# Jordy-VL/multi-modal-early-exit

Hardware: NVIDIA B200
Metric: docs/sec @ calibrated exit threshold (higher is better)
Workload: dtype bf16

## Files before the change

multi-modal-early-exit_b200/csrc/attention.cuh:

```cuda
#pragma once
#include <cuda.h>

#include <type_traits>

#include "ptx.cuh"

namespace mmee {

constexpr int ATT_SM_WARPS = 4;
constexpr int ATT_THREADS = 64 + ATT_SM_WARPS * 32;
constexpr int ATT_CTAS_PER_SM = 2;
constexpr int ATT_BQ = 128;
constexpr int ATT_BKV = 64;
constexpr int ATT_D = 64;
constexpr int ATT_DV = 80;
constexpr int ATT_KB_STAGES = 2;
constexpr int ATT_V_STAGES = 2;
constexpr int ATT_MAX_KV_TILES = 16;
constexpr float ATT_LAZY = 8.0f;
constexpr float ATT_JUMP = 40.0f;

template <bool kSplit>
struct AttSmemT {
  static constexpr int NP = kSplit ? 2 : 1;
  static constexpr int Q_BYTES = ATT_BQ * ATT_D * 2;
  static constexpr int K_BYTES = ATT_BKV * ATT_D * 2;
  static constexpr int V_BYTES = ATT_DV * ATT_BKV * 2;
  static constexpr int VLO_BYTES = kSplit ? ATT_D * ATT_BKV * 2 : 0;
  static constexpr int B_BYTES = ATT_BQ * ATT_BKV * 2;
  static constexpr int Q_STAGE = NP * Q_BYTES;
  static constexpr int KB_STAGE = NP * (K_BYTES + B_BYTES);
  static constexpr int V_STAGE = V_BYTES + VLO_BYTES;
  static constexpr int I_BYTES = ATT_BKV * ATT_BKV * 2;
  static constexpr int Q_OFF = 0;
  static constexpr int KB_OFF = Q_OFF + 2 * Q_STAGE;
  static constexpr int V_OFF = KB_OFF + ATT_KB_STAGES * KB_STAGE;
  static constexpr int I_OFF = V_OFF + ATT_V_STAGES * V_STAGE;
  static constexpr int BAR_OFF = I_OFF + I_BYTES;
  static constexpr int N_BARS = 2 + 2 + 2 * ATT_KB_STAGES + 2 * ATT_V_STAGES + 2 + 2 + 1 + 1;
  static constexpr int TOTAL = BAR_OFF + N_BARS * 8 + 16;
  static constexpr int DYN_BYTES = TOTAL;
  static constexpr uint32_t TMEM_COLS = kSplit ? 512 : 256;
};
using AttSmem = AttSmemT<false>;
static_assert(AttSmem::DYN_BYTES <= 115712, "two attention CTAs must fit one SM");
static_assert(AttSmemT<true>::DYN_BYTES <= 232448, "split attention CTA must fit one SM");
static_assert(AttSmem::KB_STAGE % 1024 == 0 && AttSmem::K_BYTES % 1024 == 0 && AttSmem::V_BYTES % 1024 == 0 &&
                  AttSmem::V_OFF % 1024 == 0 && AttSmem::I_OFF % 1024 == 0 && AttSmemT<true>::V_STAGE % 1024 == 0 &&
                  AttSmemT<true>::V_OFF % 1024 == 0 && AttSmemT<true>::I_OFF % 1024 == 0,
              "swizzled tiles need 1024 B alignment");

struct AttArgs {
  const int4* slot_meta;
  const int* qt_slot;
  const int* n_qt_dev;
  int* err_flag;
  long long* trace;
  __nv_bfloat16* ctx;
  __nv_bfloat16* ctx_lo;
  int H, heads, seq;
  int tail16;
  int experiment;
};

__device__ __forceinline__ float fast_exp2(float x) {
  float y;
  asm("ex2.approx.ftz.f32 %0, %1;" : "=f"(y) : "f"(x));
  return y;
}

__device__ __forceinline__ void sub_ref_x2(uint32_t a, uint32_t b, uint64_t nref2, float& ya, float& yb) {
  uint64_t x, y;
  asm("mov.b64 %0, {%1, %2};" : "=l"(x) : "r"(a), "r"(b));
  asm("add.rn.f32x2 %0, %1, %2;" : "=l"(y) : "l"(x), "l"(nref2));
  asm("mov.b64 {%0, %1}, %2;" : "=f"(ya), "=f"(yb) : "l"(y));
}

// ... 16 lines not shown
  c.nitem = total_items;
  if (!c.valid) return c;
  c.row0 = meta.x; c.rows = meta.y; c.doc = meta.z;
  const int n_qt = (c.rows + ATT_BQ - 1) / ATT_BQ;
  const int local = item - args.heads * meta.w;
  c.head = local / n_qt;
  c.q0 = (local - c.head * n_qt) * ATT_BQ;
  c.slot = __ldg(args.qt_slot + item / args.heads);
  c.last_j = (c.rows + ATT_BKV - 1) / ATT_BKV - 1;
  const int rem = c.rows - c.last_j * ATT_BKV;
  c.tail_j = (args.tail16 && c.last_j > 0 && rem <= 16) ? c.last_j : -1;
  c.nitem = item + stride;
  c.nmeta = att_item_meta(c.nitem, total_items, args);
  return c;
}
__device__ __forceinline__ AttCursor att_first(int total_items, int stride, const AttArgs& args) {
  const int item = blockIdx.x;
  return att_enter(item, 0, att_item_meta(item, total_items, args), total_items, stride, args);
}
__device__ __forceinline__ AttCursor att_next(AttCursor c, int total_items, int stride, const AttArgs& args) {
  if (c.j < c.last_j) { ++c.j; return c; }
  return att_enter(c.nitem, c.ii + 1, c.nmeta, total_items, stride, args);
}

struct AttMaps {
  CUtensorMap q, k, vt, bias, q_lo, k_lo, vt_lo, bias_lo;
};

template <bool kTrace, bool kSplit = false>
__global__ void __launch_bounds__(ATT_THREADS, kSplit ? 1 : ATT_CTAS_PER_SM)
attention_kernel(const __grid_constant__ AttMaps maps, const AttArgs args) {
  using SMEM = AttSmemT<kSplit>;
  const CUtensorMap& tmap_q = maps.q;
  const CUtensorMap& tmap_k = maps.k;
  const CUtensorMap& tmap_vt = maps.vt;
  const CUtensorMap& tmap_bias = maps.bias;
  const int S = args.seq;
  const int total_items = *args.n_qt_dev * args.heads;
  const int stride = gridDim.x;
  if (total_items == 0) return;

  extern __shared__ __align__(1024) uint8_t smem_raw[];
  const uint32_t sb = smem_u32(smem_raw);
  uint8_t* smem = smem_raw;
  if (sb & 1023u) __trap();
  const uint32_t bar0 = sb + SMEM::BAR_OFF;
  const uint32_t q_full = bar0;
  const uint32_t q_empty = q_full + 2 * 8;
  const uint32_t kb_full = q_empty + 2 * 8;
  const uint32_t kb_empty = kb_full + ATT_KB_STAGES * 8;
  const uint32_t v_full = kb_empty + ATT_KB_STAGES * 8;
  const uint32_t v_empty = v_full + ATT_V_STAGES * 8;
  const uint32_t s_full = v_empty + ATT_V_STAGES * 8;
  const uint32_t p_full = s_full + 2 * 8;
  const uint32_t o_full = p_full + 2 * 8;
  const uint32_t qt_full = o_full + 8;
  uint64_t* bars = reinterpret_cast<uint64_t*>(smem + SMEM::BAR_OFF);
  uint32_t* tmem_slot = reinterpret_cast<uint32_t*>(bars + SMEM::N_BARS);

  const int warp = threadIdx.x >> 5;
  const int lane = threadIdx.x & 31;
#define ATT_TRACE(R, T, K)                                                                             \
  if constexpr (kTrace) {                                                                              \
    if (blockIdx.x == 0 && (T) < 96) args.trace[(R) * 1024 + (T) * 8 + (K)] = clock64();              \
  }

  if (warp == 0 && lane == 0) {
    tma_prefetch_desc(&tmap_q);
    tma_prefetch_desc(&tmap_k);
    tma_prefetch_desc(&tmap_vt);
    tma_prefetch_desc(&tmap_bias);
    if constexpr (kSplit) {
      tma_prefetch_desc(&maps.q_lo); tma_prefetch_desc(&maps.k_lo); tma_prefetch_desc(&maps.vt_lo); tma_prefetch_desc(&maps.bias_lo);
    }
    uint64_t* b = bars;
    for (int i = 0; i < 2; ++i) mbar_init(b++, 1);
    for (int i = 0; i < 2; ++i) mbar_init(b++, ATT_SM_WARPS);
    for (int i = 0; i < 2 * ATT_KB_STAGES; ++i) mbar_init(b++, 1);
    for (int i = 0; i < 2 * ATT_V_STAGES; ++i) mbar_init(b++, 1);
    for (int i = 0; i < 2; ++i) mbar_init(b++, 1);
    for (int i = 0; i < 2; ++i) mbar_init(b++, ATT_SM_WARPS);
    mbar_init(b++, 1);
    mbar_init(b++, ATT_SM_WARPS);
    fence_mbar_init();
  }
  for (int i = threadIdx.x; i < ATT_V_STAGES * 128; i += blockDim.x) {
    const int stg = i >> 7, chunk = i & 127;
    uint8_t* base = smem + SMEM::V_OFF + stg * SMEM::V_STAGE + ATT_D * 128;
    const uint32_t val = (chunk < 8) ? 0x3F803F80u : 0u;
    *reinterpret_cast<uint4*>(base + chunk * 16) = make_uint4(val, val, val, val);
  }
  for (int i = threadIdx.x; i < ATT_BKV * 8; i += blockDim.x) {
    const int n = i >> 3, cchunk = i & 7;
    uint32_t w[4] = {0u, 0u, 0u, 0u};
    if ((n >> 3) == cchunk) w[(n & 7) >> 1] = (n & 1) ? 0x3C000000u : 0x00003C00u;
    *reinterpret_cast<uint4*>(smem + SMEM::I_OFF + n * 128 + ((cchunk ^ (n & 7)) << 4)) = make_uint4(w[0], w[1], w[2], w[3]);
  }
  fence_proxy_async_smem();
  if (warp == 1) tmem_alloc<SMEM::TMEM_COLS>(tmem_slot);
  tc_fence_before();
  __syncthreads();
  tc_fence_after();
  const uint32_t tmem_base = *tmem_slot;
  const uint32_t tmem_S = tmem_base;
  const uint32_t tmem_O = tmem_base + 128;
  const uint32_t tmem_Q = tmem_base + 208;
  const uint32_t tmem_Qlo = tmem_base + 240;

  if (warp == 0) {
    if (elect_one()) {
      AttCursor c = att_first(total_items, stride, args);
      uint32_t t = 0;
      int loaded_ii = -1;
      int pv_row = 0, pv_kv0 = 0;
      constexpr int PF_DIST = 4;
      while (c.valid) {
        const int row0 = c.row0;
        if (c.ii != loaded_ii) {
          loaded_ii = c.ii;
          auto load_q = [&](int k, int qrow, int qhead) {
            const int qb = k & 1;
            mbar_wait(q_empty + qb * 8, ((k >> 1) & 1) ^ 1);
            mbar_expect_tx(q_full + qb * 8, SMEM::Q_STAGE);
            tma_load_2d(sb + SMEM::Q_OFF + qb * SMEM::Q_STAGE, &tmap_q, q_full + qb * 8, qhead * ATT_D, qrow);
            if constexpr (kSplit)
              tma_load_2d(sb + SMEM::Q_OFF + qb * SMEM::Q_STAGE + SMEM::Q_BYTES, &maps.q_lo, q_full + qb * 8, qhead * ATT_D, qrow);
          };
          ATT_TRACE(2, t, 2)
          if (c.ii == 0) load_q(0, row0 + c.q0, c.head);
          if (c.nitem < total_items) {
            const int nn_qt = (c.nmeta.y + ATT_BQ - 1) / ATT_BQ;
            const int nlocal = c.nitem - args.heads * c.nmeta.w;
            const int nhead = nlocal / nn_qt;
            load_q(c.ii + 1, c.nmeta.x + (nlocal - nhead * nn_qt) * ATT_BQ, nhead);
          }
        }
        const int kv0 = c.j * ATT_BKV;
        const int brow = (c.doc * args.heads + c.head) * S + c.q0;
        const int vrow = (c.slot * args.heads + c.head) * ATT_D;
        const int st = t % ATT_KB_STAGES;
        ATT_TRACE(2, t, 0)
        mbar_wait(kb_empty + st * 8, ((t / ATT_KB_STAGES) & 1) ^ 1);
        ATT_TRACE(2, t, 1)
        const uint32_t sk = sb + SMEM::KB_OFF + st * SMEM::KB_STAGE;
        if (!kSplit && args.experiment && t >= 4) {
          const uint32_t bytes = ((args.experiment & 1) ? 0 : SMEM::K_BYTES) + ((args.experiment & 2) ? 0 : SMEM::B_BYTES);
          if (bytes) mbar_expect_tx(kb_full + st * 8, bytes); else mbar_arrive(kb_full + st * 8);
          if (!(args.experiment & 1)) tma_load_2d(sk, &tmap_k, kb_full + st * 8, args.H + c.head * ATT_D, row0 + kv0);
          if (!(args.experiment & 2)) tma_load_2d(sk + SMEM::NP * SMEM::K_BYTES, &tmap_bias, kb_full + st * 8, kv0, brow);
        } else {
        mbar_expect_tx(kb_full + st * 8, SMEM::KB_STAGE);
        tma_load_2d(sk, &tmap_k, kb_full + st * 8, args.H + c.head * ATT_D, row0 + kv0);
        tma_load_2d(sk + SMEM::NP * SMEM::K_BYTES, &tmap_bias, kb_full + st * 8, kv0, brow);
        }
        if constexpr (kSplit) {
          tma_load_2d(sk + SMEM::K_BYTES, &maps.k_lo, kb_full + st * 8, args.H + c.head * ATT_D, row0 + kv0);
          tma_load_2d(sk + 2 * SMEM::K_BYTES + SMEM::B_BYTES, &maps.bias_lo, kb_full + st * 8, kv0, brow);
        }
        {
// ... 16 lines not shown
            }
          }
          if (pj <= plast) {
            tma_prefetch_2d(&tmap_bias, pj * ATT_BKV, pbrow);
            tma_prefetch_2d(&tmap_k, args.H + phead * ATT_D, prow0 + pj * ATT_BKV);
            tma_prefetch_2d(&tmap_vt, pj * ATT_BKV, pvrow);
          }
        }
        if (t > 0) {
          const int sv = (t - 1) % ATT_V_STAGES;
          mbar_wait(v_empty + sv * 8, (((t - 1) / ATT_V_STAGES) & 1) ^ 1);
          if (!kSplit && (args.experiment & 1) && t >= 4) {
            mbar_arrive(v_full + sv * 8);
          } else {
          mbar_expect_tx(v_full + sv * 8, SMEM::NP * ATT_D * ATT_BKV * 2);
          tma_load_2d(sb + SMEM::V_OFF + sv * SMEM::V_STAGE, &tmap_vt, v_full + sv * 8, pv_kv0, pv_row);
          if constexpr (kSplit)
            tma_load_2d(sb + SMEM::V_OFF + sv * SMEM::V_STAGE + SMEM::V_BYTES, &maps.vt_lo, v_full + sv * 8, pv_kv0, pv_row);
          }
        }
        pv_row = vrow; pv_kv0 = kv0;
        ++t;
        c = att_next(c, total_items, stride, args);
      }
      if (t > 0) {
        const int sv = (t - 1) % ATT_V_STAGES;
        mbar_wait(v_empty + sv * 8, (((t - 1) / ATT_V_STAGES) & 1) ^ 1);
        mbar_expect_tx(v_full + sv * 8, SMEM::NP * ATT_D * ATT_BKV * 2);
        tma_load_2d(sb + SMEM::V_OFF + sv * SMEM::V_STAGE, &tmap_vt, v_full + sv * 8, pv_kv0, pv_row);
        if constexpr (kSplit)
          tma_load_2d(sb + SMEM::V_OFF + sv * SMEM::V_STAGE + SMEM::V_BYTES, &maps.vt_lo, v_full + sv * 8, pv_kv0, pv_row);
      }
    }
  } else if (warp == 1) {
    if (elect_one()) {
      constexpr uint32_t idesc_s = umma_idesc_bf16(ATT_BQ, ATT_BKV);
      constexpr uint32_t idesc_o = umma_idesc_bf16(ATT_BQ, ATT_DV);
      constexpr uint32_t idesc_s16 = umma_idesc_bf16(ATT_BQ, 16);
      constexpr uint32_t idesc_b16 = umma_idesc_f16(ATT_BQ, 16);
      const uint64_t di = umma_desc_sw128_kmajor(sb + SMEM::I_OFF);
      AttCursor cs = att_first(total_items, stride, args);
      AttCursor cp = cs;
      uint32_t ts = 0;
      auto issue_s = [&]() {
        const int st = ts % ATT_KB_STAGES;
        ATT_TRACE(1, ts, 0)
        if (cs.j == 0) mbar_wait(qt_full, cs.ii & 1);
        mbar_wait(kb_full + st * 8, (ts / ATT_KB_STAGES) & 1);
        ATT_TRACE(1, ts, 1)
        tc_fence_after();
        const uint32_t stage = sb + SMEM::KB_OFF + st * SMEM::KB_STAGE;
        const uint64_t dk = umma_desc_sw128_kmajor(stage);
        const uint64_t db = umma_desc_sw128_kmajor(stage + SMEM::NP * SMEM::K_BYTES);
        const uint32_t d_s = tmem_S + (ts & 1) * ATT_BKV;
        if constexpr (kSplit) {
          const uint64_t dkl = umma_desc_sw128_kmajor(stage + SMEM::K_BYTES);
          const uint64_t dbl = umma_desc_sw128_kmajor(stage + 2 * SMEM::K_BYTES + SMEM::B_BYTES);
#pragma unroll
          for (int k = 0; k < ATT_D / 16; ++k) umma_bf16_ts(d_s, tmem_Q + k * 8, dk + 2 * k, idesc_s, k ? 1u : 0u);
#pragma unroll
          for (int k = 0; k < ATT_D / 16; ++k) umma_bf16_ts(d_s, tmem_Qlo + k * 8, dk + 2 * k, idesc_s, 1u);
#pragma unroll
          for (int k = 0; k < ATT_D / 16; ++k) umma_bf16_ts(d_s, tmem_Q + k * 8, dkl + 2 * k, idesc_s, 1u);
#pragma unroll
          for (int k = 0; k < ATT_BKV / 16; ++k) umma_bf16_ss(d_s + 16 * k, db + 2 * k, di + 130 * k, idesc_b16, 1u);
#pragma unroll
// ... 12 lines not shown
        umma_commit(kb_empty + st * 8);
        ++ts;
        cs = att_next(cs, total_items, stride, args);
      };
      if (cs.valid) issue_s();
      for (uint32_t t = 0; t < ts; ++t) {
        if (cs.valid) issue_s();
        const int sv = t % ATT_V_STAGES;
        const int b = t & 1;
        const bool first = (cp.j == 0);
        ATT_TRACE(1, t, 2)
        mbar_wait(p_full + b * 8, (t >> 1) & 1);
        ATT_TRACE(1, t, 3)
        mbar_wait(v_full + sv * 8, (t / ATT_V_STAGES) & 1);
        tc_fence_after();
        const uint64_t dv = umma_desc_sw128_kmajor(sb + SMEM::V_OFF + sv * SMEM::V_STAGE);
        const int pv_steps = (kSplit || cp.j != cp.tail_j) ? ATT_BKV / 16 : 1;
#pragma unroll
        for (int k = 0; k < ATT_BKV / 16; ++k)
          if (k < pv_steps)
            umma_bf16_ts(tmem_O, tmem_S + b * ATT_BKV + k * 8, dv + 2 * k, idesc_o, (k || !first) ? 1u : 0u);
        if constexpr (kSplit) {
          constexpr uint32_t idesc_o64 = umma_idesc_bf16(ATT_BQ, ATT_D);
          const uint64_t dvl = umma_desc_sw128_kmajor(sb + SMEM::V_OFF + sv * SMEM::V_STAGE + SMEM::V_BYTES);
#pragma unroll
          for (int k = 0; k < ATT_BKV / 16; ++k) umma_bf16_ts(tmem_O, tmem_S + b * ATT_BKV + 32 + k * 8, dv + 2 * k, idesc_o, 1u);
#pragma unroll
          for (int k = 0; k < ATT_BKV / 16; ++k) umma_bf16_ts(tmem_O, tmem_S + b * ATT_BKV + k * 8, dvl + 2 * k, idesc_o64, 1u);
        }
        umma_commit(o_full);
        umma_commit(v_empty + sv * 8);
        cp = att_next(cp, total_items, stride, args);
      }
    }
  } else {
    const int quarter = warp & 3;
    const int r = quarter * 32 + lane;
    const uint32_t lane_addr = static_cast<uint32_t>(quarter * 32) << 16;
    uint32_t t = 0;
    AttCursor c = att_first(total_items, stride, args);

    float ref = 0.f, alpha_pend = 1.f;
    __nv_bfloat16* out_ptr = nullptr;
    bool have_item = false;

    auto store_item = [&](__nv_bfloat16* dst_row) {
      uint32_t v[32];
      const uint32_t lsum = tmem_ld1(tmem_O + lane_addr + ATT_D);
      tmem_ld32(tmem_O + lane_addr, v);
      tmem_ld_wait();
      const float inv = 1.0f / __uint_as_float(lsum);
      if constexpr (kSplit) {
        __nv_bfloat16* lo_row = dst_row ? args.ctx_lo + (dst_row - args.ctx) : nullptr;
#pragma unroll
        for (int hh = 0; hh < 2; ++hh) {
// ... 28 lines not shown
      tmem_ld32(tmem_O + lane_addr + 32, v);
      tmem_ld_wait();
      if (dst_row) {
#pragma unroll
        for (int i = 0; i < 4; ++i)
          dst[4 + i] = make_uint4(pack_bf16x2(__uint_as_float(v[i * 8 + 0]) * inv, __uint_as_float(v[i * 8 + 1]) * inv),
                                  pack_bf16x2(__uint_as_float(v[i * 8 + 2]) * inv, __uint_as_float(v[i * 8 + 3]) * inv),
                                  pack_bf16x2(__uint_as_float(v[i * 8 + 4]) * inv, __uint_as_float(v[i * 8 + 5]) * inv),
                                  pack_bf16x2(__uint_as_float(v[i * 8 + 6]) * inv, __uint_as_float(v[i * 8 + 7]) * inv));
      }
    };

    auto q_to_tmem = [&](int ii) {
      const int qb = ii & 1;
      mbar_wait(q_full + qb * 8, (ii >> 1) & 1);
      const uint32_t qrow = sb + SMEM::Q_OFF + qb * SMEM::Q_STAGE + r * 128;
      uint32_t q[32];
#pragma unroll
      for (int cch = 0; cch < 8; ++cch) {
        const uint4 x = lds128(qrow + ((cch ^ (r & 7)) << 4));
        q[4 * cch] = x.x; q[4 * cch + 1] = x.y; q[4 * cch + 2] = x.z; q[4 * cch + 3] = x.w;
      }
      tmem_st32(tmem_Q + lane_addr, q);
      if constexpr (kSplit) {
#pragma unroll
        for (int cch = 0; cch < 8; ++cch) {
          const uint4 x = lds128(qrow + SMEM::Q_BYTES + ((cch ^ (r & 7)) << 4));
          q[4 * cch] = x.x; q[4 * cch + 1] = x.y; q[4 * cch + 2] = x.z; q[4 * cch + 3] = x.w;
        }
        tmem_st32(tmem_Qlo + lane_addr, q);
      }
// ... 1 lines not shown
      tc_fence_before();
      __syncwarp();
      if (lane == 0) { mbar_arrive(qt_full); mbar_arrive(q_empty + qb * 8); }
    };
    if (c.valid) q_to_tmem(0);

    while (c.valid) {
      const int b = t & 1;
      const bool first = (c.j == 0);
      const uint32_t tS = tmem_S + lane_addr + b * ATT_BKV;
      __nv_bfloat16* prev_out = out_ptr;
      if (first) {
        const int q = c.q0 + r;
        out_ptr = (q < c.rows) ? args.ctx + static_cast<size_t>(c.row0 + q) * args.H + c.head * ATT_D : nullptr;
      }
      const bool tr = kTrace && warp == 2 && lane == 0;
      if (tr) { ATT_TRACE(0, t, 0) }
      mbar_wait(s_full + b * 8, (t >> 1) & 1);
      tc_fence_after();
      if (tr) { ATT_TRACE(0, t, 1) }
      if (c.j == c.last_j && c.nitem < total_items) q_to_tmem(c.ii + 1);

      float pmax;
      if constexpr (kSplit) {
        uint32_t v0[32], v1[32], ph[32], pl[32];
        tmem_ld32(tS, v0);
        tmem_ld32(tS + 32, v1);
        tmem_ld_wait();
        if (first) {
          float m0 = fmaxf(__uint_as_float(v0[0]), __uint_as_float(v0[1]));
#pragma unroll
// ... 21 lines not shown
          pmax -= dq;
#pragma unroll
          for (int i = 0; i < 32; ++i) {
            const float e0 = fast_exp2(__uint_as_float(i < 16 ? v0[2 * i] : v1[2 * i - 32]) - ref);
            const float e1 = fast_exp2(__uint_as_float(i < 16 ? v0[2 * i + 1] : v1[2 * i - 31]) - ref);
            ph[i] = pack_bf16x2(e0, e1);
            const float2 hf = unpack_bf16x2(ph[i]);
            pl[i] = pack_bf16x2(e0 - hf.x, e1 - hf.y);
          }
        }
        __syncwarp();
        tmem_st32(tS, ph);
        tmem_st32(tS + 32, pl);
      } else if (c.j == c.tail_j) {
        uint32_t v[16], pq[8];
        tmem_ld16(tS, v);
        tmem_ld_wait();
        if (tr) { ATT_TRACE(0, t, 2) }
        if (first) {
          float m = fmaxf(__uint_as_float(v[0]), __uint_as_float(v[1]));
#pragma unroll
          for (int i = 2; i < 16; i += 2) m = fmaxf(m, fmaxf(__uint_as_float(v[i]), __uint_as_float(v[i + 1])));
          ref = m;
        }
        float m = -INFINITY;
#pragma unroll
        for (int i = 0; i < 8; ++i) {
          const float a0 = __uint_as_float(v[2 * i]) - ref, a1 = __uint_as_float(v[2 * i + 1]) - ref;
          m = fmaxf(m, fmaxf(a0, a1));
          pq[i] = pack_bf16x2(fast_exp2(a0), fast_exp2(a1));
// ... 4 lines not shown
          ref += dq;
          alpha_pend *= fast_exp2(-dq);
          pmax -= dq;
#pragma unroll
          for (int i = 0; i < 8; ++i)
            pq[i] = pack_bf16x2(fast_exp2(__uint_as_float(v[2 * i]) - ref), fast_exp2(__uint_as_float(v[2 * i + 1]) - ref));
        }
        __syncwarp();
        tmem_st8(tS, pq);
      } else {
        uint32_t v0[32], v1[32], pk[32];
        tmem_ld32(tS, v0);
        tmem_ld32(tS + 32, v1);
        tmem_ld_wait();
        if (tr) { ATT_TRACE(0, t, 2) }
        if (first) {
          float m0 = fmaxf(__uint_as_float(v0[0]), __uint_as_float(v0[1]));
          float m1 = fmaxf(__uint_as_float(v1[0]), __uint_as_float(v1[1]));
#pragma unroll
          for (int i = 2; i < 32; i += 2) {
            m0 = fmaxf(m0, fmaxf(__uint_as_float(v0[i]), __uint_as_float(v0[i + 1])));
            m1 = fmaxf(m1, fmaxf(__uint_as_float(v1[i]), __uint_as_float(v1[i + 1])));
          }
          ref = fmaxf(m0, m1);
          pmax = 0.f;
        }
        {
          float m0 = -INFINITY, m1 = -INFINITY;
          uint64_t nref2;
          asm("mov.b64 %0, {%1, %1};" : "=l"(nref2) : "f"(-ref));
// ... 11 lines not shown
        }
        if (pmax > ATT_JUMP) {
          const float dq = ceilf(pmax);
          ref += dq;
          alpha_pend *= fast_exp2(-dq);
          pmax -= dq;
#pragma unroll
          for (int i = 0; i < 16; ++i) {
            pk[i] = pack_bf16x2(fast_exp2(__uint_as_float(v0[2 * i]) - ref), fast_exp2(__uint_as_float(v0[2 * i + 1]) - ref));
            pk[16 + i] = pack_bf16x2(fast_exp2(__uint_as_float(v1[2 * i]) - ref), fast_exp2(__uint_as_float(v1[2 * i + 1]) - ref));
          }
        }
        __syncwarp();
        tmem_st32(tS, pk);
      }
      if (tr) { ATT_TRACE(0, t, 3) }

      if (t > 0) {
        mbar_wait(o_full, (t - 1) & 1);
        tc_fence_after();
        if (tr) { ATT_TRACE(0, t, 4) }
        if (first) {
          if (have_item) store_item(prev_out);
        } else if (__any_sync(0xffffffffu, alpha_pend != 1.0f)) {
          uint32_t o[32];
#pragma unroll
          for (int hh = 0; hh < 2; ++hh) {
            tmem_ld32(tmem_O + lane_addr + hh * 32, o);
            tmem_ld_wait();
#pragma unroll
// ... 15 lines not shown
      alpha_pend = 1.f;
      if (pmax > ATT_LAZY) {
        const float dq = ceilf(pmax);
        ref += dq;
        alpha_pend = fast_exp2(-dq);
        if (!(alpha_pend > 0.f)) *args.err_flag = 1;
      }
      ++t;
      c = att_next(c, total_items, stride, args);
    }
    if (have_item) {
      mbar_wait(o_full, (t - 1) & 1);
      tc_fence_after();
      store_item(out_ptr);
    }
  }

#undef ATT_TRACE
  tc_fence_before();
  __syncthreads();
  if (warp == 1) {
    tc_fence_after();
    tmem_dealloc<SMEM::TMEM_COLS>(tmem_base);
  }
}

}
```

multi-modal-early-exit_b200/csrc/engine.cu:

```cuda
#include <cuda.h>
#include <cuda_runtime.h>
#include <math.h>
#include <stdint.h>
#include <stdlib.h>
#include <string.h>

#include <algorithm>
#include <map>
#include <memory>
#include <numeric>
#include <stdexcept>
#include <string>
#include <vector>

#include "../../include/mmee.h"
#include "attention.cuh"
#include "embed.cuh"
#include "gemm.cuh"
#include "norm_exit.cuh"
#include "policy.cuh"
#include "calibrate.cuh"
#include "tmap.h"

using namespace mmee;
// ... 589 lines not shown
  e->t_bias = make_tmap_2d_sw128(e->BIAS.p, static_cast<uint64_t>(B) * heads * S, e->bias_width, e->bias_pitch, ATT_BQ,
                                 CU_TENSOR_MAP_DATA_TYPE_FLOAT16);
  e->n_kv_tiles = (S + ATT_BKV - 1) / ATT_BKV;
  if (e->n_kv_tiles > ATT_MAX_KV_TILES) throw std::runtime_error("too many key tiles");
  e->maskadd.alloc(static_cast<size_t>(B) * e->kv_pitch, true);
  e->err_flags.alloc(2, true);
  e->doc_len.alloc(B, true);
  e->kept_idx.alloc(static_cast<size_t>(B) * std::max(e->T, 1), true);
  const int max_qt = (S + ATT_BQ - 1) / ATT_BQ;
  for (int i = 0; i < 2; ++i) {
    e->plan_row0[i].alloc(B + 1, true);
    e->plan_meta[i].alloc(B, true);
    e->plan_qt_slot[i].alloc(static_cast<size_t>(B) * max_qt, true);
    e->plan_n_qt[i].alloc(1, true);
  }
  e->att_trace.alloc(4096, true);
  e->t_ctx = make_tmap_2d_sw128(e->CTX.p, M, H, H, 128);
  e->t_a1 = make_tmap_2d_sw128(e->A1.p, M, H, H, 128);
  e->t_mid = make_tmap_2d_sw128(e->MID.p, M, I, I, 128);
  e->t_patch = make_tmap_2d_sw128(e->PATCH.p, mp, e->kdim_patch, e->kdim_patch, 128);
  if (e->split) {
    e->t_x_lo[0] = make_tmap_2d_sw128(e->Xlo[0].p, M, H, H, 128);
    e->t_x_lo[1] = make_tmap_2d_sw128(e->Xlo[1].p, M, H, H, 128);
    e->t_qk_lo = make_tmap_2d_sw128(e->QKlo.p, M, 2 * H, 2 * H, 128);
    e->t_k64_lo = make_tmap_2d_sw128(e->QKlo.p, M, 2 * H, 2 * H, ATT_BKV);
    e->t_vt_lo = make_tmap_2d_sw128(e->VTlo.p, static_cast<uint64_t>(B) * heads * 64, e->kv_pitch, e->kv_pitch, 64);
    e->t_bias_lo = make_tmap_2d_sw128(e->BIASlo.p, static_cast<uint64_t>(B) * heads * S, e->bias_width, e->bias_pitch, ATT_BQ,
                                      CU_TENSOR_MAP_DATA_TYPE_FLOAT16);
    e->t_ctx_lo = make_tmap_2d_sw128(e->CTXlo.p, M, H, H, 128);
    e->t_a1_lo = make_tmap_2d_sw128(e->A1lo.p, M, H, H, 128);
    e->t_mid_lo = make_tmap_2d_sw128(e->MIDlo.p, M, I, I, 128);
// ... 378 lines not shown
  for (int l = 0; l < e->L; ++l) {
    LayerW& w = e->layers[l];
    const int* mdev = e->m_dev.p + stage;
    GemmArgs ga{};
    ga.m_dev = mdev; ga.N = 3 * H; ga.K = H; ga.bias = w.bqkv.p; ga.out = e->QK.p; ga.out_lo = e->QKlo.p; ga.ld_out = 2 * H;
    ga.vt = e->VT.p; ga.vt_lo = e->VTlo.p; ga.qk_cols = 2 * H; ga.row0 = e->plan_row0[rp].p; ga.n_slots_dev = e->n_dev.p + stage;
    ga.kv_pitch = e->kv_pitch; ga.heads = heads;
    launch_gemm<EPI_QKV>(e, e->bn_qkv, e->t_x[cur], w.t_wqkv, ga, st, &e->t_x_lo[cur], &w.t_wqkv_lo);
    mark(e, "gemm", st);

    AttArgs aa;
    aa.slot_meta = e->plan_meta[rp].p; aa.qt_slot = e->plan_qt_slot[rp].p; aa.n_qt_dev = e->plan_n_qt[rp].p;
    aa.ctx = e->CTX.p; aa.ctx_lo = e->CTXlo.p; aa.H = H; aa.heads = heads; aa.seq = S;
    aa.tail16 = (e->tail16 && !split) ? 1 : 0;
    aa.experiment = getenv("MMEE_ATT_EXPERIMENT") ? atoi(getenv("MMEE_ATT_EXPERIMENT")) : 0; aa.err_flag = e->err_flags.p; aa.trace = e->att_trace.p;
    {
      static bool configured_dev[64] = {};
      bool& configured = configured_dev[e->device & 63];
      if (!configured) {
        CUDA_OK(cudaFuncSetAttribute(attention_kernel<false, false>, cudaFuncAttributeMaxDynamicSharedMemorySize, AttSmem::DYN_BYTES + 16 * 1024));
        CUDA_OK(cudaFuncSetAttribute(attention_kernel<true, false>, cudaFuncAttributeMaxDynamicSharedMemorySize, AttSmem::DYN_BYTES + 16 * 1024));
        CUDA_OK(cudaFuncSetAttribute(attention_kernel<false, true>, cudaFuncAttributeMaxDynamicSharedMemorySize, AttSmemT<true>::DYN_BYTES));
        configured = true;
      }
      AttMaps am;
      am.q = e->t_qk; am.k = e->t_k64; am.vt = e->t_vt; am.bias = e->t_bias;
      if (split) { am.q_lo = e->t_qk_lo; am.k_lo = e->t_k64_lo; am.vt_lo = e->t_vt_lo; am.bias_lo = e->t_bias_lo; }
      else { am.q_lo = e->t_qk; am.k_lo = e->t_k64; am.vt_lo = e->t_vt; am.bias_lo = e->t_bias; }
      static const bool one_cta = getenv("MMEE_ATT_ONE_CTA") != nullptr;
      const int att_grid = e->sms * ((split || one_cta) ? 1 : ATT_CTAS_PER_SM);
      const size_t att_smem = AttSmem::DYN_BYTES + (one_cta ? 16 * 1024 : 0);
      if (split)
        attention_kernel<false, true><<<att_grid, ATT_THREADS, AttSmemT<true>::DYN_BYTES, st>>>(am, aa);
      else if (e->trace_on && l == 0)
        attention_kernel<true, false><<<att_grid, ATT_THREADS, att_smem, st>>>(am, aa);
      else
        attention_kernel<false, false><<<att_grid, ATT_THREADS, att_smem, st>>>(am, aa);
      CUDA_OK(cudaGetLastError());
      e->launches++;
    }
    mark(e, "attention", st);

    const bool yr = e->y_resid;
    static const int resid_pf = getenv("MMEE_RESID_PREFETCH") ? atoi(getenv("MMEE_RESID_PREFETCH")) : 0;
    float* y_att = yr ? e->Y2.p : e->Y.p;
    ga = GemmArgs{};
    ga.m_dev = mdev; ga.N = H; ga.K = H; ga.bias = w.bo.p; ga.out = y_att; ga.ld_out = H; ga.resid = e->X[cur].p;
    ga.resid_lo = (x_lo_valid && !yr) ? e->Xlo[cur].p : nullptr;
    ga.resid_f32 = split ? e->X32[cur].p : nullptr;
    if (yr && x_lo_valid) {
      const LayerW& pw = e->layers[l - 1];
      ga.resid = nullptr; ga.resid_prefetch = resid_pf;
// ... 906 lines not shown
```

Baseline: 8920.

## Merge two attention CTAs into one CTA with two pipelines and softmax token handover

Replaces two independent attention CTAs per SM with a single CTA that runs two complete producer/MMA/softmax pipelines, each with its own smem region, barriers and half of a 512-column TMEM allocation. The two pipelines' softmax warpgroups pass a token through named barriers so that their exp phases alternate rather than compete for the SFU/ALU, with a finish flag so one pipeline can stop waiting once the other is done. The aim is to overlap one pipeline's softmax with the other's MMA/TMA work. The cost is extra named-barrier synchronisation and coupling between the pipelines, so a stalled pipeline can hold up its partner.

```diff
diff --git a/multi-modal-early-exit_b200/csrc/attention.cuh b/multi-modal-early-exit_b200/csrc/attention.cuh
--- a/multi-modal-early-exit_b200/csrc/attention.cuh
+++ b/multi-modal-early-exit_b200/csrc/attention.cuh
@@ -8,7 +8,8 @@
 namespace mmee {
 
 constexpr int ATT_SM_WARPS = 4;
-constexpr int ATT_THREADS = 64 + ATT_SM_WARPS * 32;
+constexpr int ATT_PIPE_WARPS = 2 + ATT_SM_WARPS;
+constexpr int ATT_THREADS = ATT_PIPE_WARPS * 32;
 constexpr int ATT_CTAS_PER_SM = 2;
 constexpr int ATT_BQ = 128;
 constexpr int ATT_BKV = 64;
@@ -22,6 +23,8 @@
 
 template <bool kSplit>
 struct AttSmemT {
+  static constexpr int NPIPE = kSplit ? 1 : 2;
+  static constexpr int THREADS = NPIPE * ATT_THREADS;
   static constexpr int NP = kSplit ? 2 : 1;
   static constexpr int Q_BYTES = ATT_BQ * ATT_D * 2;
   static constexpr int K_BYTES = ATT_BKV * ATT_D * 2;
@@ -35,19 +38,21 @@
   static constexpr int Q_OFF = 0;
   static constexpr int KB_OFF = Q_OFF + 2 * Q_STAGE;
   static constexpr int V_OFF = KB_OFF + ATT_KB_STAGES * KB_STAGE;
-  static constexpr int I_OFF = V_OFF + ATT_V_STAGES * V_STAGE;
+  static constexpr int PIPE_BYTES = V_OFF + ATT_V_STAGES * V_STAGE;
+  static constexpr int I_OFF = NPIPE * PIPE_BYTES;
   static constexpr int BAR_OFF = I_OFF + I_BYTES;
   static constexpr int N_BARS = 2 + 2 + 2 * ATT_KB_STAGES + 2 * ATT_V_STAGES + 2 + 2 + 1 + 1;
-  static constexpr int TOTAL = BAR_OFF + N_BARS * 8 + 16;
+  static constexpr int TOTAL = BAR_OFF + NPIPE * N_BARS * 8 + 16;
   static constexpr int DYN_BYTES = TOTAL;
-  static constexpr uint32_t TMEM_COLS = kSplit ? 512 : 256;
+  static constexpr uint32_t TMEM_COLS = 512;
+  static constexpr uint32_t TMEM_PIPE = 256;
 };
 using AttSmem = AttSmemT<false>;
-static_assert(AttSmem::DYN_BYTES <= 115712, "two attention CTAs must fit one SM");
-static_assert(AttSmemT<true>::DYN_BYTES <= 232448, "split attention CTA must fit one SM");
+static_assert(AttSmem::DYN_BYTES <= 232448 && AttSmemT<true>::DYN_BYTES <= 232448, "an attention CTA must fit one SM");
 static_assert(AttSmem::KB_STAGE % 1024 == 0 && AttSmem::K_BYTES % 1024 == 0 && AttSmem::V_BYTES % 1024 == 0 &&
-                  AttSmem::V_OFF % 1024 == 0 && AttSmem::I_OFF % 1024 == 0 && AttSmemT<true>::V_STAGE % 1024 == 0 &&
-                  AttSmemT<true>::V_OFF % 1024 == 0 && AttSmemT<true>::I_OFF % 1024 == 0,
+                  AttSmem::V_OFF % 1024 == 0 && AttSmem::PIPE_BYTES % 1024 == 0 && AttSmem::I_OFF % 1024 == 0 &&
+                  AttSmemT<true>::V_STAGE % 1024 == 0 && AttSmemT<true>::V_OFF % 1024 == 0 &&
+                  AttSmemT<true>::I_OFF % 1024 == 0,
               "swizzled tiles need 1024 B alignment");
 
 struct AttArgs {
@@ -61,6 +66,7 @@
   int H, heads, seq;
   int tail16;
   int experiment;
+  int no_handover;
 };
 
 __device__ __forceinline__ float fast_exp2(float x) {
@@ -107,8 +113,7 @@
   c.nmeta = att_item_meta(c.nitem, total_items, args);
   return c;
 }
-__device__ __forceinline__ AttCursor att_first(int total_items, int stride, const AttArgs& args) {
-  const int item = blockIdx.x;
+__device__ __forceinline__ AttCursor att_first(int item, int total_items, int stride, const AttArgs& args) {
   return att_enter(item, 0, att_item_meta(item, total_items, args), total_items, stride, args);
 }
 __device__ __forceinline__ AttCursor att_next(AttCursor c, int total_items, int stride, const AttArgs& args) {
@@ -116,12 +121,28 @@
   return att_enter(c.nitem, c.ii + 1, c.nmeta, total_items, stride, args);
 }
 
+struct AttToken {
+  volatile int* fin;
+  int pipe;
+  bool fin_prev;
+
+  __device__ __forceinline__ void take() const { asm volatile("bar.sync %0, 256;" ::"r"(1 + pipe) : "memory"); }
+  __device__ __forceinline__ bool end_turn(bool done) {
+    const bool other = fin[pipe ^ 1] != 0;
+    if (other && fin_prev) return true;
+    if (done && !fin_prev && (threadIdx.x & 127) == 0) fin[pipe] = 1;
+    fin_prev = done;
+    asm volatile("bar.arrive %0, 256;" ::"r"(2 - pipe) : "memory");
+    return done && other;
+  }
+};
+
 struct AttMaps {
   CUtensorMap q, k, vt, bias, q_lo, k_lo, vt_lo, bias_lo;
 };
 
 template <bool kTrace, bool kSplit = false>
-__global__ void __launch_bounds__(ATT_THREADS, kSplit ? 1 : ATT_CTAS_PER_SM)
+__global__ void __launch_bounds__(AttSmemT<kSplit>::THREADS, 1)
 attention_kernel(const __grid_constant__ AttMaps maps, const AttArgs args) {
   using SMEM = AttSmemT<kSplit>;
   const CUtensorMap& tmap_q = maps.q;
@@ -130,14 +151,21 @@
   const CUtensorMap& tmap_bias = maps.bias;
   const int S = args.seq;
   const int total_items = *args.n_qt_dev * args.heads;
-  const int stride = gridDim.x;
+  const int npipe = kSplit ? 1 : blockDim.x / ATT_THREADS;
+  const int stride = gridDim.x * npipe;
   if (total_items == 0) return;
 
   extern __shared__ __align__(1024) uint8_t smem_raw[];
   const uint32_t sb = smem_u32(smem_raw);
   uint8_t* smem = smem_raw;
   if (sb & 1023u) __trap();
-  const uint32_t bar0 = sb + SMEM::BAR_OFF;
+  const int warp = threadIdx.x >> 5;
+  const int lane = threadIdx.x & 31;
+  const int pipe = warp / ATT_PIPE_WARPS;
+  const int role = warp - pipe * ATT_PIPE_WARPS;
+  const int item0 = blockIdx.x * npipe + pipe;
+  const uint32_t sp = sb + pipe * SMEM::PIPE_BYTES;
+  const uint32_t bar0 = sb + SMEM::BAR_OFF + pipe * SMEM::N_BARS * 8;
   const uint32_t q_full = bar0;
   const uint32_t q_empty = q_full + 2 * 8;
   const uint32_t kb_full = q_empty + 2 * 8;
@@ -149,13 +177,12 @@
   const uint32_t o_full = p_full + 2 * 8;
   const uint32_t qt_full = o_full + 8;
   uint64_t* bars = reinterpret_cast<uint64_t*>(smem + SMEM::BAR_OFF);
-  uint32_t* tmem_slot = reinterpret_cast<uint32_t*>(bars + SMEM::N_BARS);
-
-  const int warp = threadIdx.x >> 5;
-  const int lane = threadIdx.x & 31;
+  uint32_t* tmem_slot = reinterpret_cast<uint32_t*>(bars + SMEM::NPIPE * SMEM::N_BARS);
+  volatile int* token_fin = reinterpret_cast<volatile int*>(tmem_slot + 1);
+
 #define ATT_TRACE(R, T, K)                                                                             \
   if constexpr (kTrace) {                                                                              \
-    if (blockIdx.x == 0 && (T) < 96) args.trace[(R) * 1024 + (T) * 8 + (K)] = clock64();              \
+    if (blockIdx.x == 0 && (T) < 96) args.trace[(pipe * 3 + (R)) * 1024 + (T) * 8 + (K)] = clock64();  \
   }
 
   if (warp == 0 && lane == 0) {
@@ -167,19 +194,24 @@
       tma_prefetch_desc(&maps.q_lo); tma_prefetch_desc(&maps.k_lo); tma_prefetch_desc(&maps.vt_lo); tma_prefetch_desc(&maps.bias_lo);
     }
     uint64_t* b = bars;
-    for (int i = 0; i < 2; ++i) mbar_init(b++, 1);
-    for (int i = 0; i < 2; ++i) mbar_init(b++, ATT_SM_WARPS);
-    for (int i = 0; i < 2 * ATT_KB_STAGES; ++i) mbar_init(b++, 1);
-    for (int i = 0; i < 2 * ATT_V_STAGES; ++i) mbar_init(b++, 1);
-    for (int i = 0; i < 2; ++i) mbar_init(b++, 1);
-    for (int i = 0; i < 2; ++i) mbar_init(b++, ATT_SM_WARPS);
-    mbar_init(b++, 1);
-    mbar_init(b++, ATT_SM_WARPS);
+    for (int p = 0; p < SMEM::NPIPE; ++p) {
+      for (int i = 0; i < 2; ++i) mbar_init(b++, 1);
+      for (int i = 0; i < 2; ++i) mbar_init(b++, ATT_SM_WARPS);
+      for (int i = 0; i < 2 * ATT_KB_STAGES; ++i) mbar_init(b++, 1);
+      for (int i = 0; i < 2 * ATT_V_STAGES; ++i) mbar_init(b++, 1);
+      for (int i = 0; i < 2; ++i) mbar_init(b++, 1);
+      for (int i = 0; i < 2; ++i) mbar_init(b++, ATT_SM_WARPS);
+      mbar_init(b++, 1);
+      mbar_init(b++, ATT_SM_WARPS);
+    }
+    token_fin[0] = 0;
+    token_fin[1] = 0;
     fence_mbar_init();
   }
-  for (int i = threadIdx.x; i < ATT_V_STAGES * 128; i += blockDim.x) {
+  for (int i = threadIdx.x; i < SMEM::NPIPE * ATT_V_STAGES * 128; i += blockDim.x) {
     const int stg = i >> 7, chunk = i & 127;
-    uint8_t* base = smem + SMEM::V_OFF + stg * SMEM::V_STAGE + ATT_D * 128;
+    uint8_t* base = smem + (stg / ATT_V_STAGES) * SMEM::PIPE_BYTES + SMEM::V_OFF + (stg % ATT_V_STAGES) * SMEM::V_STAGE +
+                    ATT_D * 128;
     const uint32_t val = (chunk < 8) ? 0x3F803F80u : 0u;
     *reinterpret_cast<uint4*>(base + chunk * 16) = make_uint4(val, val, val, val);
   }
@@ -195,14 +227,14 @@
   __syncthreads();
   tc_fence_after();
   const uint32_t tmem_base = *tmem_slot;
-  const uint32_t tmem_S = tmem_base;
-  const uint32_t tmem_O = tmem_base + 128;
-  const uint32_t tmem_Q = tmem_base + 208;
-  const uint32_t tmem_Qlo = tmem_base + 240;
-
-  if (warp == 0) {
+  const uint32_t tmem_S = tmem_base + pipe * SMEM::TMEM_PIPE;
+  const uint32_t tmem_O = tmem_S + 128;
+  const uint32_t tmem_Q = tmem_S + 208;
+  const uint32_t tmem_Qlo = tmem_S + 240;
+
+  if (role == 0) {
     if (elect_one()) {
-      AttCursor c = att_first(total_items, stride, args);
+      AttCursor c = att_first(item0, total_items, stride, args);
       uint32_t t = 0;
       int loaded_ii = -1;
       int pv_row = 0, pv_kv0 = 0;
@@ -215,9 +247,9 @@
             const int qb = k & 1;
             mbar_wait(q_empty + qb * 8, ((k >> 1) & 1) ^ 1);
             mbar_expect_tx(q_full + qb * 8, SMEM::Q_STAGE);
-            tma_load_2d(sb + SMEM::Q_OFF + qb * SMEM::Q_STAGE, &tmap_q, q_full + qb * 8, qhead * ATT_D, qrow);
+            tma_load_2d(sp + SMEM::Q_OFF + qb * SMEM::Q_STAGE, &tmap_q, q_full + qb * 8, qhead * ATT_D, qrow);
             if constexpr (kSplit)
-              tma_load_2d(sb + SMEM::Q_OFF + qb * SMEM::Q_STAGE + SMEM::Q_BYTES, &maps.q_lo, q_full + qb * 8, qhead * ATT_D, qrow);
+              tma_load_2d(sp + SMEM::Q_OFF + qb * SMEM::Q_STAGE + SMEM::Q_BYTES, &maps.q_lo, q_full + qb * 8, qhead * ATT_D, qrow);
           };
           ATT_TRACE(2, t, 2)
           if (c.ii == 0) load_q(0, row0 + c.q0, c.head);
@@ -235,7 +267,7 @@
         ATT_TRACE(2, t, 0)
         mbar_wait(kb_empty + st * 8, ((t / ATT_KB_STAGES) & 1) ^ 1);
         ATT_TRACE(2, t, 1)
-        const uint32_t sk = sb + SMEM::KB_OFF + st * SMEM::KB_STAGE;
+        const uint32_t sk = sp + SMEM::KB_OFF + st * SMEM::KB_STAGE;
         if (!kSplit && args.experiment && t >= 4) {
           const uint32_t bytes = ((args.experiment & 1) ? 0 : SMEM::K_BYTES) + ((args.experiment & 2) ? 0 : SMEM::B_BYTES);
           if (bytes) mbar_expect_tx(kb_full + st * 8, bytes); else mbar_arrive(kb_full + st * 8);
@@ -282,9 +314,9 @@
             mbar_arrive(v_full + sv * 8);
           } else {
           mbar_expect_tx(v_full + sv * 8, SMEM::NP * ATT_D * ATT_BKV * 2);
-          tma_load_2d(sb + SMEM::V_OFF + sv * SMEM::V_STAGE, &tmap_vt, v_full + sv * 8, pv_kv0, pv_row);
+          tma_load_2d(sp + SMEM::V_OFF + sv * SMEM::V_STAGE, &tmap_vt, v_full + sv * 8, pv_kv0, pv_row);
           if constexpr (kSplit)
-            tma_load_2d(sb + SMEM::V_OFF + sv * SMEM::V_STAGE + SMEM::V_BYTES, &maps.vt_lo, v_full + sv * 8, pv_kv0, pv_row);
+            tma_load_2d(sp + SMEM::V_OFF + sv * SMEM::V_STAGE + SMEM::V_BYTES, &maps.vt_lo, v_full + sv * 8, pv_kv0, pv_row);
           }
         }
         pv_row = vrow; pv_kv0 = kv0;
@@ -295,19 +327,19 @@
         const int sv = (t - 1) % ATT_V_STAGES;
         mbar_wait(v_empty + sv * 8, (((t - 1) / ATT_V_STAGES) & 1) ^ 1);
         mbar_expect_tx(v_full + sv * 8, SMEM::NP * ATT_D * ATT_BKV * 2);
-        tma_load_2d(sb + SMEM::V_OFF + sv * SMEM::V_STAGE, &tmap_vt, v_full + sv * 8, pv_kv0, pv_row);
+        tma_load_2d(sp + SMEM::V_OFF + sv * SMEM::V_STAGE, &tmap_vt, v_full + sv * 8, pv_kv0, pv_row);
         if constexpr (kSplit)
-          tma_load_2d(sb + SMEM::V_OFF + sv * SMEM::V_STAGE + SMEM::V_BYTES, &maps.vt_lo, v_full + sv * 8, pv_kv0, pv_row);
+          tma_load_2d(sp + SMEM::V_OFF + sv * SMEM::V_STAGE + SMEM::V_BYTES, &maps.vt_lo, v_full + sv * 8, pv_kv0, pv_row);
       }
     }
-  } else if (warp == 1) {
+  } else if (role == 1) {
     if (elect_one()) {
       constexpr uint32_t idesc_s = umma_idesc_bf16(ATT_BQ, ATT_BKV);
       constexpr uint32_t idesc_o = umma_idesc_bf16(ATT_BQ, ATT_DV);
       constexpr uint32_t idesc_s16 = umma_idesc_bf16(ATT_BQ, 16);
       constexpr uint32_t idesc_b16 = umma_idesc_f16(ATT_BQ, 16);
       const uint64_t di = umma_desc_sw128_kmajor(sb + SMEM::I_OFF);
-      AttCursor cs = att_first(total_items, stride, args);
+      AttCursor cs = att_first(item0, total_items, stride, args);
       AttCursor cp = cs;
       uint32_t ts = 0;
       auto issue_s = [&]() {
@@ -317,7 +349,7 @@
         mbar_wait(kb_full + st * 8, (ts / ATT_KB_STAGES) & 1);
         ATT_TRACE(1, ts, 1)
         tc_fence_after();
-        const uint32_t stage = sb + SMEM::KB_OFF + st * SMEM::KB_STAGE;
+        const uint32_t stage = sp + SMEM::KB_OFF + st * SMEM::KB_STAGE;
         const uint64_t dk = umma_desc_sw128_kmajor(stage);
         const uint64_t db = umma_desc_sw128_kmajor(stage + SMEM::NP * SMEM::K_BYTES);
         const uint32_t d_s = tmem_S + (ts & 1) * ATT_BKV;
@@ -360,7 +392,7 @@
         ATT_TRACE(1, t, 3)
         mbar_wait(v_full + sv * 8, (t / ATT_V_STAGES) & 1);
         tc_fence_after();
-        const uint64_t dv = umma_desc_sw128_kmajor(sb + SMEM::V_OFF + sv * SMEM::V_STAGE);
+        const uint64_t dv = umma_desc_sw128_kmajor(sp + SMEM::V_OFF + sv * SMEM::V_STAGE);
         const int pv_steps = (kSplit || cp.j != cp.tail_j) ? ATT_BKV / 16 : 1;
 #pragma unroll
         for (int k = 0; k < ATT_BKV / 16; ++k)
@@ -368,7 +400,7 @@
             umma_bf16_ts(tmem_O, tmem_S + b * ATT_BKV + k * 8, dv + 2 * k, idesc_o, (k || !first) ? 1u : 0u);
         if constexpr (kSplit) {
           constexpr uint32_t idesc_o64 = umma_idesc_bf16(ATT_BQ, ATT_D);
-          const uint64_t dvl = umma_desc_sw128_kmajor(sb + SMEM::V_OFF + sv * SMEM::V_STAGE + SMEM::V_BYTES);
+          const uint64_t dvl = umma_desc_sw128_kmajor(sp + SMEM::V_OFF + sv * SMEM::V_STAGE + SMEM::V_BYTES);
 #pragma unroll
           for (int k = 0; k < ATT_BKV / 16; ++k) umma_bf16_ts(tmem_O, tmem_S + b * ATT_BKV + 32 + k * 8, dv + 2 * k, idesc_o, 1u);
 #pragma unroll
@@ -384,7 +416,11 @@
     const int r = quarter * 32 + lane;
     const uint32_t lane_addr = static_cast<uint32_t>(quarter * 32) << 16;
     uint32_t t = 0;
-    AttCursor c = att_first(total_items, stride, args);
+    AttCursor c = att_first(item0, total_items, stride, args);
+    const bool handover = npipe == 2 && !args.no_handover;
+    AttToken token{token_fin, pipe, false};
+    bool token_left = false;
+    if (handover && pipe == 1) token_left = token.end_turn(!c.valid);
 
     float ref = 0.f, alpha_pend = 1.f;
     __nv_bfloat16* out_ptr = nullptr;
@@ -443,7 +479,7 @@
     auto q_to_tmem = [&](int ii) {
       const int qb = ii & 1;
       mbar_wait(q_full + qb * 8, (ii >> 1) & 1);
-      const uint32_t qrow = sb + SMEM::Q_OFF + qb * SMEM::Q_STAGE + r * 128;
+      const uint32_t qrow = sp + SMEM::Q_OFF + qb * SMEM::Q_STAGE + r * 128;
       uint32_t q[32];
 #pragma unroll
       for (int cch = 0; cch < 8; ++cch) {
@@ -475,7 +511,7 @@
         const int q = c.q0 + r;
         out_ptr = (q < c.rows) ? args.ctx + static_cast<size_t>(c.row0 + q) * args.H + c.head * ATT_D : nullptr;
       }
-      const bool tr = kTrace && warp == 2 && lane == 0;
+      const bool tr = kTrace && role == 2 && lane == 0;
       if (tr) { ATT_TRACE(0, t, 0) }
       mbar_wait(s_full + b * 8, (t >> 1) & 1);
       tc_fence_after();
@@ -527,6 +563,8 @@
         tmem_st32(tS + 32, pl);
       } else if (c.j == c.tail_j) {
         uint32_t v[16], pq[8];
+        if (handover) token.take();
+        if (tr) { ATT_TRACE(0, t, 6) }
         tmem_ld16(tS, v);
         tmem_ld_wait();
         if (tr) { ATT_TRACE(0, t, 2) }
@@ -561,6 +599,8 @@
         tmem_ld32(tS + 32, v1);
         tmem_ld_wait();
         if (tr) { ATT_TRACE(0, t, 2) }
+        if (handover) token.take();
+        if (tr) { ATT_TRACE(0, t, 6) }
         if (first) {
           float m0 = fmaxf(__uint_as_float(v0[0]), __uint_as_float(v0[1]));
           float m1 = fmaxf(__uint_as_float(v1[0]), __uint_as_float(v1[1]));
@@ -602,6 +642,7 @@
         __syncwarp();
         tmem_st32(tS, pk);
       }
+      if (handover) token_left = token.end_turn(c.j == c.last_j && c.nitem >= total_items);
       if (tr) { ATT_TRACE(0, t, 3) }
 
       if (t > 0) {
@@ -647,6 +688,10 @@
       tc_fence_after();
       store_item(out_ptr);
     }
+    while (handover && !token_left) {
+      token.take();
+      token_left = token.end_turn(true);
+    }
   }
 
 #undef ATT_TRACE
diff --git a/multi-modal-early-exit_b200/csrc/engine.cu b/multi-modal-early-exit_b200/csrc/engine.cu
--- a/multi-modal-early-exit_b200/csrc/engine.cu
+++ b/multi-modal-early-exit_b200/csrc/engine.cu
@@ -627,7 +627,7 @@
     e->plan_qt_slot[i].alloc(static_cast<size_t>(B) * max_qt, true);
     e->plan_n_qt[i].alloc(1, true);
   }
-  e->att_trace.alloc(4096, true);
+  e->att_trace.alloc(8192, true);
   e->t_ctx = make_tmap_2d_sw128(e->CTX.p, M, H, H, 128);
   e->t_a1 = make_tmap_2d_sw128(e->A1.p, M, H, H, 128);
   e->t_mid = make_tmap_2d_sw128(e->MID.p, M, I, I, 128);
@@ -1036,12 +1036,14 @@
     aa.ctx = e->CTX.p; aa.ctx_lo = e->CTXlo.p; aa.H = H; aa.heads = heads; aa.seq = S;
     aa.tail16 = (e->tail16 && !split) ? 1 : 0;
     aa.experiment = getenv("MMEE_ATT_EXPERIMENT") ? atoi(getenv("MMEE_ATT_EXPERIMENT")) : 0; aa.err_flag = e->err_flags.p; aa.trace = e->att_trace.p;
+    static const bool no_handover = getenv("MMEE_ATT_NO_HANDOVER") != nullptr;
+    aa.no_handover = no_handover ? 1 : 0;
     {
       static bool configured_dev[64] = {};
       bool& configured = configured_dev[e->device & 63];
       if (!configured) {
-        CUDA_OK(cudaFuncSetAttribute(attention_kernel<false, false>, cudaFuncAttributeMaxDynamicSharedMemorySize, AttSmem::DYN_BYTES + 16 * 1024));
-        CUDA_OK(cudaFuncSetAttribute(attention_kernel<true, false>, cudaFuncAttributeMaxDynamicSharedMemorySize, AttSmem::DYN_BYTES + 16 * 1024));
+        CUDA_OK(cudaFuncSetAttribute(attention_kernel<false, false>, cudaFuncAttributeMaxDynamicSharedMemorySize, AttSmem::DYN_BYTES));
+        CUDA_OK(cudaFuncSetAttribute(attention_kernel<true, false>, cudaFuncAttributeMaxDynamicSharedMemorySize, AttSmem::DYN_BYTES));
         CUDA_OK(cudaFuncSetAttribute(attention_kernel<false, true>, cudaFuncAttributeMaxDynamicSharedMemorySize, AttSmemT<true>::DYN_BYTES));
         configured = true;
       }
@@ -1049,15 +1051,13 @@
       am.q = e->t_qk; am.k = e->t_k64; am.vt = e->t_vt; am.bias = e->t_bias;
       if (split) { am.q_lo = e->t_qk_lo; am.k_lo = e->t_k64_lo; am.vt_lo = e->t_vt_lo; am.bias_lo = e->t_bias_lo; }
       else { am.q_lo = e->t_qk; am.k_lo = e->t_k64; am.vt_lo = e->t_vt; am.bias_lo = e->t_bias; }
-      static const bool one_cta = getenv("MMEE_ATT_ONE_CTA") != nullptr;
-      const int att_grid = e->sms * ((split || one_cta) ? 1 : ATT_CTAS_PER_SM);
-      const size_t att_smem = AttSmem::DYN_BYTES + (one_cta ? 16 * 1024 : 0);
+      const int att_grid = e->sms;
       if (split)
-        attention_kernel<false, true><<<att_grid, ATT_THREADS, AttSmemT<true>::DYN_BYTES, st>>>(am, aa);
+        attention_kernel<false, true><<<att_grid, AttSmemT<true>::THREADS, AttSmemT<true>::DYN_BYTES, st>>>(am, aa);
       else if (e->trace_on && l == 0)
-        attention_kernel<true, false><<<att_grid, ATT_THREADS, att_smem, st>>>(am, aa);
+        attention_kernel<true, false><<<att_grid, AttSmem::THREADS, AttSmem::DYN_BYTES, st>>>(am, aa);
       else
-        attention_kernel<false, false><<<att_grid, ATT_THREADS, att_smem, st>>>(am, aa);
+        attention_kernel<false, false><<<att_grid, AttSmem::THREADS, AttSmem::DYN_BYTES, st>>>(am, aa);
       CUDA_OK(cudaGetLastError());
       e->launches++;
     }
diff --git a/profiles/att_trace_pipelines.py b/profiles/att_trace_pipelines.py
--- /dev/null
+++ b/profiles/att_trace_pipelines.py
@@ -0,0 +1,44 @@
+import os, sys
+import numpy as np, torch
+ROOT = os.path.dirname(os.path.dirname(os.path.abspath(__file__)))
+sys.path.insert(0, ROOT); sys.path.insert(0, os.path.join(ROOT, "multi-modal-early-exit_b200"))
+from mmee import synth
+from mmee.config import ExitConfig, ModelDims
+from mmee.model import B200EEForSequenceClassification
+
+n = int(sys.argv[1]) if len(sys.argv) > 1 else 256
+dims = ModelDims.base(layers=1)
+ee = ExitConfig.from_dict(dict(exits=["text_visual_concat", 1], encoder_layer_strategy="ramp", inference_strategy="max_confidence"))
+sd = synth.make_state_dict(dims, ee, seed=0)
+docs = synth.make_docs(dims, n, seed=3, pad=False)
+model = B200EEForSequenceClassification(dims, ee, sd, device=0, max_batch=n)
+dev = {k: v.cuda() for k, v in docs.items()}
+model.forward(**dev); torch.cuda.synchronize()
+model._lib.mmee_set_profiling(model._h, 2)
+model.forward(**dev); torch.cuda.synchronize()
+tr = model.debug_read("ATT_TRACE", np.int64, 8192)
+blk = lambda p, role: tr[(p * 3 + role) * 1024:(p * 3 + role) * 1024 + 768].reshape(96, 8)
+t0 = min(int(blk(p, 0)[0, 0]) for p in range(2) if blk(p, 0)[0, 0])
+for p in range(2):
+    sm = blk(p, 0)
+    print(f"=== pipeline {p}: softmax warp 2 | tile @start | s_full wait, tmem ld, token wait, exp+st, o_full wait, "
+          f"fence+arrive | tile period | exp phase @start .. @end")
+    for t in range(1, 50):
+        r = sm[t]
+        if r[0] == 0: break
+        d4 = r[4] if r[4] else r[3]
+        tok = r[6] if r[6] else r[2]
+        start = max(tok, r[2])
+        print(f"{t:3d} @{r[0]-t0:8d} | {r[1]-r[0]:6d} {r[2]-r[1]:6d} {max(tok-r[2], 0):6d} {r[3]-start:6d} "
+              f"{d4-r[3]:6d} {r[5]-d4:6d} | {sm[t+1,0]-r[0] if sm[t+1,0] else 0:6d} | @{start-t0:8d} .. @{r[3]-t0:8d}")
+ph = []
+for p in range(2):
+    sm = blk(p, 0)
+    for t in range(1, 96):
+        r = sm[t]
+        if r[0] == 0: break
+        ph.append((max(r[6] if r[6] else r[2], r[2]) - t0, r[3] - t0, p))
+ph.sort()
+ov = sum(max(0, min(a[1], b[1]) - b[0]) for a, b in zip(ph, ph[1:]) if a[2] != b[2])
+print(f"exp phases in time order (pipeline of each): {''.join(str(x[2]) for x in ph[:60])}")
+print(f"cycles in which the two pipelines' exp phases overlap: {ov} of {ph[-1][1] - ph[0][0]}")
```

New measurement: 8763, median of 6. -1.8%, worse.
